# cg-tuwien/ppsurf

Hardware: AMD Instinct MI355X
Metric: occupancy query-points/sec @ res=257, 50NN (higher is better)
Workload: dtype f16x3

## Files before the change

ppsurf_amd/csrc/pps_decode.hip:

```cpp
#include <cstdlib>
#include "pps_common.h"
#include "../../include/ppsurf_amd.h"

using namespace pps;

#define NT 256
#define NW (NT / 64)
#define WG_PER_CU (512 / NT)
#ifndef PPS_PRIO
#define PPS_PRIO 1
#endif
#ifndef PPS_PRIO_PN
#define PPS_PRIO_PN 1
#endif
#define CH4 2048

template <int CHUNK_F4_NEXT, int NTH = NT, class F>
__device__ __forceinline__ void stream_step(const f32x4* __restrict__ gnext, f32x4*& cur, f32x4*& nxt, F&& compute) {
    chunk_copy_async<CHUNK_F4_NEXT / NTH, NTH>(gnext, nxt);
    compute((const f32x4*)cur);
    stream_wait();
    wg_barrier();
    f32x4* t = cur; cur = nxt; nxt = t;
}
// ... 773 lines not shown

#define PB_NBIAS (128 + 64 + 4096)
#define PB_LDS_BYTES (2 * CH4 * 16 + 4096 * 4)

__global__ __launch_bounds__(NT, 2) void pointnet_stn_fc_kernel(const float* __restrict__ gin, int64_t Q,
                                                                const float* __restrict__ wpack, const float* __restrict__ bias,
                                                                float* __restrict__ trans2, const int* __restrict__ gate) {
    if (gate_closed(gate)) return;
    float* bias_l = (float*)((f32x4*)pps_smem + 2 * CH4);
    const f32x4* bias4 = (const f32x4*)bias_l;
    const f32x4* wg = (const f32x4*)wpack;
    const int lane = lane_id(), wave = threadIdx.x >> 6, n = lane & 15, g = lane >> 4;

    lds_fill(bias_l, bias + 192, 4096);
    const f32x4* bias_g = (const f32x4*)bias;
    f32x4 *cur, *nxt;
    stream_begin<CH4>(wg, cur, nxt);

    const int ntiles = (int)((Q + NW * 16 - 1) / (NW * 16));
    int first, count, stride;
    xcd_tile_range(ntiles, first, count, stride);
    for (int it = 0; it < count; ++it) {
        const TileRow q = tile_row(first + it * stride, wave, n, Q);
        f32x4 a[16], h[8], u[4];
        {
            const f32x4* src = (const f32x4*)(gin + q.c * 256) + g;
#pragma unroll
            for (int bb = 0; bb < 16; ++bb) a[bb] = src[4 * bb];
        }
#pragma unroll
        for (int c = 0; c < 4; ++c)
            stream_step<CH4>(wg + (c + 1) * CH4, cur, nxt,
                           [&](const f32x4* w) { dense_blocks<16, 2, 1>(a, &h[2 * c], w, bias_g + 8 * c, lane); });
        stream_step<CH4>(wg + 5 * CH4, cur, nxt, [&](const f32x4* w) { dense_blocks<8, 4, 1>(h, u, w, bias_g + 32, lane); });
        f32x4* dst = (f32x4*)(trans2 + q.c * 4096) + g;
#pragma unroll 1
        for (int c = 0; c < 32; ++c) {
            f32x4 o[8];
            const f32x4* gn = (c + 1 < 32) ? wg + (6 + c) * CH4 : wg;
            stream_step<CH4>(gn, cur, nxt, [&](const f32x4* w) { dense_blocks<4, 8, 0>(u, o, w, bias4 + 32 * c, lane); });
            if (q.valid) {
#pragma unroll
                for (int j = 0; j < 8; ++j) dst[4 * (8 * c + j)] = o[j];
            }
        }
    }
}

__device__ __forceinline__ void stn_head_h(const float* __restrict__ grow, const f32x4* wg, const f32x4* after, const f32x4* __restrict__ bias_g,
                                           f32x4*& cur, f32x4*& nxt, int lane, float& amax, HiLo (&u)[2]) {
    HiLo ah[8], h[4];
    {
        f32x4 a[16];
        const f32x4* src = (const f32x4*)grow + (lane >> 4);
#pragma unroll
        for (int bb = 0; bb < 16; ++bb) a[bb] = src[4 * bb];
#pragma unroll
        for (int kb = 0; kb < 8; ++kb) ah[kb] = split_f16_r(amax, a[2 * kb], a[2 * kb + 1]);
    }
#pragma unroll
    for (int c = 0; c < 4; ++c)
        stream_step<CH4>(wg + (c + 1) * CH4, cur, nxt, [&](const f32x4* w) {
            dense_blocks_f16x3<8, 2, 1>(ah, (const half8*)w, bias_g + 8 * c, lane, [&](int, const f32x4& o0, const f32x4& o1) { h[c] = split_f16_r(amax, o0, o1); }); });
    stream_step<CH4>(after, cur, nxt, [&](const f32x4* w) {
        dense_blocks_f16x3<4, 4, 1>(h, (const half8*)w, bias_g + 32, lane, [&](int i, const f32x4& o0, const f32x4& o1) { u[i] = split_f16_r(amax, o0, o1); }); });
}

__global__ __launch_bounds__(NT, 2) void pointnet_stn_fc_h_kernel(const float* __restrict__ gin, int64_t Q, const f32x4* __restrict__ w16,
                                                                  const float* __restrict__ bias, half8* __restrict__ trans2h, int* __restrict__ range) {
    float amax = 0.f;
    float* bias_l = (float*)((f32x4*)pps_smem + 2 * CH4);
    const f32x4* bias4 = (const f32x4*)bias_l;
    const f32x4* wg = w16;
    const int lane = lane_id(), wave = threadIdx.x >> 6, n = lane & 15, g = lane >> 4;

    lds_fill(bias_l, bias + 192, 4096);
    const f32x4* bias_g = (const f32x4*)bias;
    f32x4 *cur, *nxt;
    stream_begin<CH4>(wg, cur, nxt);
    const int ntiles = (int)((Q + NW * 16 - 1) / (NW * 16));
    int first, count, stride;
    xcd_tile_range(ntiles, first, count, stride);
    for (int it = 0; it < count; ++it) {
        const TileRow q = tile_row(first + it * stride, wave, n, Q);
        HiLo u[2];
        stn_head_h(gin + q.c * 256, wg, wg + 5 * CH4, bias_g, cur, nxt, lane, amax, u);
        half8* dst = trans2h + q.c * 1024 + g;
#pragma unroll 1
        for (int c = 0; c < 32; ++c) {
            const f32x4* gn = (c + 1 < 32) ? wg + (6 + c) * CH4 : wg;
            stream_step<CH4>(gn, cur, nxt, [&](const f32x4* w) {
                dense_blocks_f16x3<2, 8, 0, false>(u, (const half8*)w, bias4 + 32 * c, lane, [&](int i, const f32x4& o0, const f32x4& o1) {
                    const int a = 2 * c + (i >> 1), kb = i & 1;
                    const HiLo v = split_f16_r(amax, o0, o1);
                    if (q.valid) {
                        half8* d = dst + (((a >> 4) * 2 + kb) * 2) * 64 + 4 * (a & 15);
                        d[0] = v.hi;
                        d[64] = v.lo;
                    }
                }); });
        }
    }
    range_commit(amax, range);
}

#define PC_W_XYZ 256
#define PC_NBIAS (576 + 256 + 4)
#define PC_WFLOATS (4096 + 8192)
#define PC_LDS_BYTES ((PC_WFLOATS + PC_W_XYZ + PC_NBIAS) * 4)

struct PhaseC {
    const f32x4 *w_c0b, *w_c2, *bias4, *u4;
    const float* xyz_l;
};
template <int NTH>
__device__ __forceinline__ PhaseC phase_c_setup(const float* __restrict__ wpack, const f32x4* __restrict__ wdense, const float* __restrict__ bias) {
    f32x4* w_l = (f32x4*)pps_smem;
    float* xyz_l = (float*)(w_l + PC_WFLOATS / 4);
    float* bias_l = xyz_l + PC_W_XYZ;
    for (int i = threadIdx.x; i < PC_WFLOATS / 4; i += NTH) w_l[i] = wdense[i];
    lds_fill(xyz_l, wpack, PC_W_XYZ);
    lds_fill(bias_l, bias, PC_NBIAS);
    const f32x4* bias4 = (const f32x4*)bias_l;
    return PhaseC{w_l, w_l + 1024, bias4, bias4 + 144, xyz_l};
}

template <bool H>
__device__ __forceinline__ void feat_rows_query(const float* __restrict__ patches, int64_t q, int P, int ntile_rows, const half8 (&th)[4][2],
                                                const half8 (&tl)[4][2], const f32x4 (&tf)[4][4], const PhaseC& pc, float s0, float& amax, int lane,
                                                float* __restrict__ xbar) {
    const int n = lane & 15, g = lane >> 4;
    const f32x4 *bias4 = pc.bias4, *u4 = pc.u4, *w_c0b = pc.w_c0b, *w_c2 = pc.w_c2;
    const float* xyz_l = pc.xyz_l;
    f32x4 acc[8];
    float mrun = -INFINITY, ssum = 0.f;
#pragma unroll
    for (int bb = 0; bb < 8; ++bb) acc[bb] = f32x4{0.f, 0.f, 0.f, 0.f};
    for (int rb = 0; rb < ntile_rows; ++rb) {
        const int rowi = rb * 16 + n;
        const bool valid = rowi < P;
        const int rowc = valid ? rowi : P - 1;
        const float coord = (g < 3) ? patches[(q * P + rowc) * 3 + g] : 0.f;
        f32x4 x0[4], y[8];
#pragma unroll
        for (int bb = 0; bb < 4; ++bb) x0[bb] = bias4[4 * bb + g];
        xyz_blocks<4>(coord, x0, xyz_l, lane);
        relu_blocks<4>(x0);
        __builtin_amdgcn_s_setprio(PPS_PRIO_PN);
        float s = 0.f;
        if (H) {
            HiLo a[2], b[2];
            a[0] = split_f16_r(amax, x0[0], x0[1]);
            a[1] = split_f16_r(amax, x0[2], x0[3]);
            dense_blocks_f16x3<2, 4, 1>(a, (const half8*)w_c0b, bias4 + 16, lane, [&](int i, const f32x4& o0, const f32x4& o1) { b[i] = split_f16_r(amax, o0, o1); });
#pragma unroll
            for (int ob = 0; ob < 4; ++ob) {
                f32x4 o = bias4[32 + 4 * ob + g], c = {0.f, 0.f, 0.f, 0.f};
#pragma unroll
                for (int kb = 0; kb < 2; ++kb) {
                    o = __builtin_amdgcn_mfma_f32_16x16x32_f16(th[ob][kb], b[kb].hi, o, 0, 0, 0);
                    c = __builtin_amdgcn_mfma_f32_16x16x32_f16(th[ob][kb], b[kb].lo, c, 0, 0, 0);
                    c = __builtin_amdgcn_mfma_f32_16x16x32_f16(tl[ob][kb], b[kb].hi, c, 0, 0, 0);
                }
                o += c;
#pragma unroll
                for (int r = 0; r < 4; ++r) x0[ob][r] = fmaxf(o[r], 0.f);
            }
            a[0] = split_f16_r(amax, x0[0], x0[1]);
            a[1] = split_f16_r(amax, x0[2], x0[3]);
            dense_blocks_f16x3<2, 8, 1>(a, (const half8*)w_c2, bias4 + 48, lane, [&](int i, const f32x4& o0, const f32x4& o1) {
                const f32x4 w0 = u4[4 * (2 * i) + g], w1 = u4[4 * (2 * i + 1) + g];
#pragma unroll
                for (int r = 0; r < 4; ++r) s += w0[r] * o0[r] + w1[r] * o1[r];
                y[2 * i] = o0;
                y[2 * i + 1] = o1;
            });
        } else {
            f32x4 x1[4];
            dense_blocks<4, 4, 1>(x0, x1, w_c0b, bias4 + 16, lane);
#pragma unroll
            for (int ob = 0; ob < 4; ++ob) {
                f32x4 o = bias4[32 + 4 * ob + g];
#pragma unroll
                for (int kb = 0; kb < 4; ++kb) {
                    o = __builtin_amdgcn_mfma_f32_16x16x4f32(tf[ob][kb].x, x1[kb].x, o, 0, 0, 0);
                    o = __builtin_amdgcn_mfma_f32_16x16x4f32(tf[ob][kb].y, x1[kb].y, o, 0, 0, 0);
                    o = __builtin_amdgcn_mfma_f32_16x16x4f32(tf[ob][kb].z, x1[kb].z, o, 0, 0, 0);
                    o = __builtin_amdgcn_mfma_f32_16x16x4f32(tf[ob][kb].w, x1[kb].w, o, 0, 0, 0);
                }
#pragma unroll
                for (int r = 0; r < 4; ++r) x0[ob][r] = fmaxf(o[r], 0.f);
            }
            dense_blocks<4, 8, 1>(x0, y, w_c2, bias4 + 48, lane);
#pragma unroll
            for (int bb = 0; bb < 8; ++bb) {
                const f32x4 w4 = u4[4 * bb + g];
#pragma unroll
                for (int r = 0; r < 4; ++r) s += w4[r] * y[bb][r];
            }
        }
        __builtin_amdgcn_s_setprio(0);
        s += shfl_xor_f32(s, 16);
        s += shfl_xor_f32(s, 32);
        s += s0;
        const float mblk = row16_max(valid ? s : -INFINITY);
        const float mnew = fmaxf(mrun, mblk);
        const float scale = __expf(mrun - mnew);
        const float en = valid ? __expf(s - mnew) : 0.f;
        mrun = mnew;
        ssum = ssum * scale + en;
#pragma unroll
        for (int bb = 0; bb < 8; ++bb)
#pragma unroll
            for (int r = 0; r < 4; ++r) acc[bb][r] = acc[bb][r] * scale + en * y[bb][r];
    }
    const float inv = 1.f / row16_sum(ssum);
    rows16_sum_transposed8(acc, lane);
    if (n < 8) ((f32x4*)(xbar + q * 128))[4 * n + g] = acc[0] * inv;
}

template <bool H>
__device__ __forceinline__ void pointnet_feat_rows_body(const float* __restrict__ patches, const float* __restrict__ trans2,
                                                        int64_t Q, int P, const float* __restrict__ wpack,
                                                        const f32x4* __restrict__ wdense, const float* __restrict__ bias,
                                                        float* __restrict__ xbar, int* __restrict__ flag) {
    if (!H && gate_closed(flag)) return;
    float amax = 0.f;
    const int lane = lane_id(), wave = threadIdx.x >> 6, n = lane & 15, g = lane >> 4;
    const PhaseC pc = phase_c_setup<PNT>(wpack, wdense, bias);
    wg_barrier();
    const float s0 = ((const float*)pc.bias4)[576 + 256];
    const int ntile_rows = (P + 15) / 16;

    const int ntiles = (int)((Q + PNW - 1) / PNW);
    int first, count, stride;
    xcd_tile_range(ntiles, first, count, stride);
    for (int it = 0; it < count; ++it) {
        const int64_t q = (int64_t)(first + it * stride) * PNW + wave;
        if (q >= Q) continue;
        half8 th[4][2], tl[4][2];
        f32x4 tf[4][4];
        if (H) {
            const half8* tq = (const half8*)trans2 + q * 1024 + 4 * n + g;
#pragma unroll
            for (int ob = 0; ob < 4; ++ob)
#pragma unroll
                for (int kb = 0; kb < 2; ++kb) { th[ob][kb] = tq[((ob * 2 + kb) * 2) * 64]; tl[ob][kb] = tq[((ob * 2 + kb) * 2 + 1) * 64]; }
        } else {
            const f32x4* tq = (const f32x4*)(trans2 + q * 4096);
#pragma unroll
            for (int ob = 0; ob < 4; ++ob)
#pragma unroll
                for (int kb = 0; kb < 4; ++kb) tf[ob][kb] = tq[(16 * ob + n) * 16 + 4 * kb + g];
        }
        feat_rows_query<H>(patches, q, P, ntile_rows, th, tl, tf, pc, s0, amax, lane, xbar);
    }
    if (H) range_commit(amax, flag);
}
template <bool H>
__global__ __launch_bounds__(PNT, 2) void pointnet_feat_rows_kernel(const float* __restrict__ patches, const float* __restrict__ trans2,
                                                                    int64_t Q, int P, const float* __restrict__ wpack,
                                                                    const f32x4* __restrict__ wdense, const float* __restrict__ bias,
                                                                    float* __restrict__ xbar, int* __restrict__ flag) {
    pointnet_feat_rows_body<H>(patches, trans2, Q, P, wpack, wdense, bias, xbar, flag);
}
template <>
PPS_PLAIN_F32
__global__ __launch_bounds__(PNT, 2) void pointnet_feat_rows_kernel<true>(const float* __restrict__ patches, const float* __restrict__ trans2,
                                                                          int64_t Q, int P, const float* __restrict__ wpack,
                                                                          const f32x4* __restrict__ wdense, const float* __restrict__ bias,
                                                                          float* __restrict__ xbar, int* __restrict__ flag) {
    pointnet_feat_rows_body<true>(patches, trans2, Q, P, wpack, wdense, bias, xbar, flag);
}

#define PH_LDS_BYTES (2 * CH4 * 16)
__global__ __launch_bounds__(NT, 2) void pointnet_stn_head_h_kernel(const float* __restrict__ gin, int64_t Q, const f32x4* __restrict__ w16,
                                                                    const float* __restrict__ bias, half8* __restrict__ uh, int* __restrict__ range) {
    float amax = 0.f;
    const f32x4* wg = w16;
    const int lane = lane_id(), wave = threadIdx.x >> 6, n = lane & 15, g = lane >> 4;
    const f32x4* bias_g = (const f32x4*)bias;
    f32x4 *cur, *nxt;
    stream_begin<CH4>(wg, cur, nxt);
    const int ntiles = (int)((Q + NW * 16 - 1) / (NW * 16));
    int first, count, stride;
    xcd_tile_range(ntiles, first, count, stride);
    for (int it = 0; it < count; ++it) {
        const TileRow q = tile_row(first + it * stride, wave, n, Q);
        HiLo u[2];
        stn_head_h(gin + q.c * 256, wg, wg, bias_g, cur, nxt, lane, amax, u);
        if (q.valid) {
            half8* dst = uh + q.c * 16 + g;
#pragma unroll
            for (int kb = 0; kb < 2; ++kb) { dst[(2 * kb) * 4] = u[kb].hi; dst[(2 * kb + 1) * 4] = u[kb].lo; }
        }
    }
    range_commit(amax, range);
}

#define PF_NT 512
#define PF_QSTRIDE 257
#define PF_BUF (8 * PF_QSTRIDE)
#define PF_LDS_BYTES (PC_LDS_BYTES + 3 * PF_BUF * 16)
PPS_PLAIN_F32
__global__ __launch_bounds__(PF_NT, 2) void pointnet_fc3_feat_rows_kernel(const float* __restrict__ patches, const half8* __restrict__ uh,
                                                                          int64_t Q, int P, const f32x4* __restrict__ wfc,
                                                                          const float* __restrict__ bias_fc, const float* __restrict__ wpack,
                                                                          const f32x4* __restrict__ wdense, const float* __restrict__ bias,
                                                                          float* __restrict__ xbar, int* __restrict__ flag) {
    float amax = 0.f;
    half8* ex = (half8*)(pps_smem + PC_LDS_BYTES);
    const int lane = lane_id(), wave = __builtin_amdgcn_readfirstlane(threadIdx.x >> 6), n = lane & 15, g = lane >> 4;
    const PhaseC pc = phase_c_setup<PF_NT>(wpack, wdense, bias);
    const float s0 = bias[576 + 256];
    const int ntile_rows = (P + 15) / 16;
    const f32x4* w3 = wfc + 5 * CH4;
    const f32x4* b3 = (const f32x4*)(bias_fc + 192);
    half8* ex_w = ex + (n < 8 ? n * PF_QSTRIDE : PF_BUF + (n - 8) * PF_QSTRIDE) + 8 * wave + g;
    const half8* ex_r = ex + wave * PF_QSTRIDE + 4 * n + g;
    const half8* ex_r2 = ex_r + PF_BUF;

    const int ntiles = (int)((Q + 15) / 16);
    int first, count, stride;
    xcd_tile_range(ntiles, first, count, stride);
    const f32x4 tf[4][4] = {};
    for (int it = 0; it < count; ++it) {
        const int64_t q0 = (int64_t)(first + it * stride) * 16;
        half8 th[4][2], tl[4][2], th2[2][2], tl2[2][2];
        {
            const int64_t qc = q0 + n < Q ? q0 + n : Q - 1;
            HiLo u[2];
#pragma unroll
            for (int kb = 0; kb < 2; ++kb) { u[kb].hi = uh[qc * 16 + (2 * kb) * 4 + g]; u[kb].lo = uh[qc * 16 + (2 * kb + 1) * 4 + g]; }
#pragma unroll
            for (int ob = 0; ob < 4; ++ob) {
                wg_barrier();
                const int c = 8 * ob + wave;
                const half8* wc = (const half8*)(w3 + c * CH4);
                asm volatile("" : "+s"(wc));
                dense_blocks_f16x3<2, 8, 0, false>(u, wc, b3 + 32 * c, lane, [&](int i, const f32x4& o0, const f32x4& o1) {
                    const HiLo v = split_f16_r(amax, o0, o1);
                    half8* d = ex_w + (n >= 8 ? (ob & 1) * PF_BUF : 0) + ((i & 1) * 2) * 64 + 4 * (i >> 1);
                    d[0] = v.hi;
                    d[64] = v.lo;
                });
                wg_barrier();
#pragma unroll
                for (int kb = 0; kb < 2; ++kb) {
                    th[ob][kb] = ex_r[(2 * kb) * 64];
                    tl[ob][kb] = ex_r[(2 * kb + 1) * 64];
                    if (ob < 2) {
                        th2[ob][kb] = ex_r2[ob * PF_BUF + (2 * kb) * 64];
                        tl2[ob][kb] = ex_r2[ob * PF_BUF + (2 * kb + 1) * 64];
                    }
                }
            }
        }
        if (q0 + wave < Q) feat_rows_query<true>(patches, q0 + wave, P, ntile_rows, th, tl, tf, pc, s0, amax, lane, xbar);
        if (q0 + wave + 8 < Q) {
#pragma unroll
            for (int kb = 0; kb < 2; ++kb) {
#pragma unroll
                for (int ob = 0; ob < 2; ++ob) {
                    th[ob][kb] = th2[ob][kb];
                    tl[ob][kb] = tl2[ob][kb];
                    th[2 + ob][kb] = ex_r2[ob * PF_BUF + (2 * kb) * 64];
                    tl[2 + ob][kb] = ex_r2[ob * PF_BUF + (2 * kb + 1) * 64];
                }
            }
            feat_rows_query<true>(patches, q0 + wave + 8, P, ntile_rows, th, tl, tf, pc, s0, amax, lane, xbar);
        }
    }
    range_commit(amax, flag);
}

#define TL_NBIAS (256 + 256 + 32)
#define TL_LDS_BYTES (2 * CH4 * 16 + TL_NBIAS * 4)

__global__ __launch_bounds__(NT, 2) void decode_tail_kernel(const float* __restrict__ pooled, const float* __restrict__ xbar, int64_t Q,
                                                            const float* __restrict__ wpack, const float* __restrict__ bias,
                                                            float* __restrict__ logits, float* __restrict__ occ, int* __restrict__ gate) {
    if (gate_closed(gate)) return;
    if (gate != nullptr && blockIdx.x == 0 && threadIdx.x == 0) atomicAdd(gate + 1, 1);
    float* bias_l = (float*)((f32x4*)pps_smem + 2 * CH4);
    const f32x4* bias4 = (const f32x4*)bias_l;
    const f32x4* wg = (const f32x4*)wpack;
    const int lane = lane_id(), wave = threadIdx.x >> 6, n = lane & 15, g = lane >> 4;

    lds_fill(bias_l, bias, TL_NBIAS);
    f32x4 *cur, *nxt;
    stream_begin<CH4>(wg, cur, nxt);

    const int ntiles = (int)((Q + NW * 16 - 1) / (NW * 16));
    int first, count, stride;
    xcd_tile_range(ntiles, first, count, stride);
    for (int it = 0; it < count; ++it) {
        const TileRow q = tile_row(first + it * stride, wave, n, Q);
        f32x4 p[16], x[8], h[16];
        {
            const f32x4* sp = (const f32x4*)(pooled + q.c * 256) + g;
            const f32x4* sx = (const f32x4*)(xbar + q.c * 128) + g;
#pragma unroll
            for (int bb = 0; bb < 16; ++bb) p[bb] = sp[4 * bb];
#pragma unroll
            for (int bb = 0; bb < 8; ++bb) x[bb] = sx[4 * bb];
        }
#pragma unroll
        for (int c = 0; c < 8; ++c)
            stream_step<CH4>(wg + (c + 1) * CH4, cur, nxt,
                           [&](const f32x4* w) { dense_blocks<16, 2, 0>(p, &h[2 * c], w, bias4 + 8 * c, lane); });
#pragma unroll
        for (int c = 0; c < 4; ++c)
            stream_step<CH4>(wg + (c + 9) * CH4, cur, nxt,
                           [&](const f32x4* w) { dense_blocks<8, 4, 1, 1>(x, &h[4 * c], w, bias4, lane); });
#pragma unroll
        for (int c = 0; c < 8; ++c)
            stream_step<CH4>(wg + (c + 13) * CH4, cur, nxt,
                           [&](const f32x4* w) { dense_blocks<16, 2, 1>(h, &p[2 * c], w, bias4 + 64 + 8 * c, lane); });
        f32x4 o[2];
        stream_step<CH4>(wg, cur, nxt, [&](const f32x4* w) { dense_blocks<16, 2, 0>(p, o, w, bias4 + 128, lane); });
        store_logits(o[0], q, g, logits, occ);
    }
}

PPS_PLAIN_F32
__global__ __launch_bounds__(NT, 2) void decode_tail_h_kernel(const float* __restrict__ pooled, const float* __restrict__ xbar, int64_t Q,
                                                              const f32x4* __restrict__ w16, const float* __restrict__ bias,
                                                              float* __restrict__ logits, float* __restrict__ occ, int* __restrict__ range) {
    float amax = 0.f;
    float* bias_l = (float*)((f32x4*)pps_smem + 2 * CH4);
    const f32x4* bias4 = (const f32x4*)bias_l;
    const f32x4* wg = w16;
    const int lane = lane_id(), wave = threadIdx.x >> 6, n = lane & 15, g = lane >> 4;

    lds_fill(bias_l, bias, TL_NBIAS);
    f32x4 *cur, *nxt;
    stream_begin<CH4>(wg, cur, nxt);

    const int ntiles = (int)((Q + NW * 16 - 1) / (NW * 16));
    int first, count, stride;
    xcd_tile_range(ntiles, first, count, stride);
    for (int it = 0; it < count; ++it) {
        const TileRow q = tile_row(first + it * stride, wave, n, Q);
        HiLo p[8], x[4];
        {
            const f32x4* sp = (const f32x4*)(pooled + q.c * 256) + g;
            const f32x4* sx = (const f32x4*)(xbar + q.c * 128) + g;
#pragma unroll
            for (int kb = 0; kb < 8; ++kb) p[kb] = split_f16_r(amax, sp[4 * (2 * kb)], sp[4 * (2 * kb + 1)]);
#pragma unroll
            for (int kb = 0; kb < 4; ++kb) x[kb] = split_f16_r(amax, sx[4 * (2 * kb)], sx[4 * (2 * kb + 1)]);
        }
        HiLo y[8];
#pragma unroll
        for (int c = 0; c < 8; ++c) {
            f32x4 h[2];
            stream_step<CH4 / 2>(wg + c * 3072 + 2048, cur, nxt, [&](const f32x4* w) {
                dense_blocks_f16x3<8, 2, 0>(p, (const half8*)w, bias4 + 8 * c, lane, [&](int, const f32x4& o0, const f32x4& o1) { h[0] = o0; h[1] = o1; }); });
            stream_step<CH4>(c + 1 < 8 ? wg + (c + 1) * 3072 : wg + 24576, cur, nxt, [&](const f32x4* w) {
                dense_blocks_f16x3<4, 2, 1, true, true>(x, (const half8*)w, bias4, lane, [&](int, const f32x4& o0, const f32x4& o1) { y[c] = split_f16_r(amax, o0, o1); }, h); });
        }
#pragma unroll
        for (int c = 0; c < 8; ++c)
            stream_step<CH4>(wg + 24576 + (c + 1) * 2048, cur, nxt, [&](const f32x4* w) {
                dense_blocks_f16x3<8, 2, 1>(y, (const half8*)w, bias4 + 64 + 8 * c, lane, [&](int, const f32x4& o0, const f32x4& o1) { p[c] = split_f16_r(amax, o0, o1); }); });
        f32x4 o[2];
        stream_step<CH4>(wg, cur, nxt, [&](const f32x4* w) {
            dense_blocks_f16x3<8, 2, 0>(p, (const half8*)w, bias4 + 128, lane, [&](int, const f32x4& o0, const f32x4& o1) { o[0] = o0; o[1] = o1; }); });
        store_logits(o[0], q, g, logits, occ);
    }
    range_commit(amax, range);
}

static int g_cu_count = 0;
static int cu_count() {
    if (g_cu_count == 0) {
        int dev = 0;
        hipDeviceProp_t prop;
        if (hipGetDevice(&dev) != hipSuccess || hipGetDeviceProperties(&prop, dev) != hipSuccess) return -1;
        g_cu_count = prop.multiProcessorCount;
    }
    return g_cu_count;
}

static int chip_wgs(int per_cu) {
    const int cus = cu_count();
    return (cus > 0 ? cus : 256) * per_cu;
}

static int grid_for(int64_t ntiles, int wgs = chip_wgs(WG_PER_CU)) {
    return (int)(ntiles < wgs ? (ntiles > 0 ? ntiles : 1) : wgs);
}

template <auto Kernel, class... Args>
static int launch(int grid, int threads, int lds, void* stream, Args... args) {
    static const bool once = lds > 0 && hipFuncSetAttribute((const void*)Kernel, hipFuncAttributeMaxDynamicSharedMemorySize, lds) == hipSuccess;
    (void)once;
    hipLaunchKernelGGL(Kernel, dim3(grid), dim3(threads), lds, (hipStream_t)stream, args...);
    return hipGetLastError() == hipSuccess ? PPS_OK : PPS_ERR_LAUNCH;
}

struct PnSplit { int64_t q_packed; int grid_packed, grid_rest, rest_mode; };
static PnSplit pn_split(int64_t q, int p) {
    const PatchPacking pk = patch_packing(p);
    PnSplit sp;
    const int wgs = chip_wgs(PN_WG_PER_CU);
    const int64_t per_round = (int64_t)wgs * PNW * pk.qg;
    sp.q_packed = pk.packed ? (q / per_round) * per_round : 0;
    if (pk.packed && getenv("PPS_PN_FORCE_PACK")) sp.q_packed = q;
    sp.grid_packed = wgs;
    sp.rest_mode = pk.packed ? 2 : 0;
    sp.grid_rest = grid_for((q - sp.q_packed + PNW - 1) / PNW, wgs);
    return sp;
}

template <bool H>
static int launch_stn_rows(const float* patches, int64_t q, int p, const float* wpack, const void* wdense, const float* bias, float* g,
                           int* flag, void* stream) {
    const PnSplit sp = pn_split(q, p);
    const char* tiles_env = getenv("PPS_STN_TILES");
    const int tmax = (tiles_env && atoi(tiles_env) == 2) ? 2 : 3;
    int rc = PPS_OK;
    if (sp.q_packed > 0)
        rc = launch<pointnet_stn_rows_kernel<H>>(sp.grid_packed, PNT, PA_LDS_BYTES, stream, patches, sp.q_packed, p, 1, tmax, wpack,
                                                 (const f32x4*)wdense, bias, g, flag);
    if (rc == PPS_OK && q > sp.q_packed)
        rc = launch<pointnet_stn_rows_kernel<H>>(sp.grid_rest, PNT, PA_LDS_BYTES, stream, patches + sp.q_packed * p * 3, q - sp.q_packed, p,
                                                 sp.rest_mode, tmax, wpack, (const f32x4*)wdense, bias, g + sp.q_packed * 256, flag);
    return rc;
}

template <bool H>
static int launch_feat_rows(const float* patches, const float* trans2, int64_t q, int p, const float* wpack, const void* wdense,
                            const float* bias, float* xbar, int* flag, void* stream) {
    return launch<pointnet_feat_rows_kernel<H>>(grid_for((q + PNW - 1) / PNW, chip_wgs(PN_WG_PER_CU)), PNT, PC_LDS_BYTES, stream, patches, trans2, q,
                                                p, wpack, (const f32x4*)wdense, bias, xbar, flag);
}

static int interp_pool_f32_impl(const float* G, const float* pts, const float* query, const int64_t* idx, int64_t q, int k,
                                const float* wpack, const float* bias, float* pooled, const int* gate, void* stream) {
    if (q < 0 || k < 1 || k > 64) return PPS_ERR_ARG;
    if (q == 0) return PPS_OK;
    if (!G || !pts || !query || !idx || !wpack || !bias || !pooled) return PPS_ERR_ARG;
    return launch<interp_pool_kernel>(grid_for((q + NW / 4 - 1) / (NW / 4)), NT, IP_LDS_BYTES, stream, G, pts, query, idx, q, k, wpack, bias, pooled,
                                      gate);
}

static int stn_fc_f32_impl(const float* g, int64_t q, const float* wpack, const float* bias, float* trans2, const int* gate, void* stream) {
    if (q < 0) return PPS_ERR_ARG;
    if (q == 0) return PPS_OK;
    if (!g || !wpack || !bias || !trans2) return PPS_ERR_ARG;
    return launch<pointnet_stn_fc_kernel>(grid_for((q + NW * 16 - 1) / (NW * 16)), NT, PB_LDS_BYTES, stream, g, q, wpack, bias, trans2, gate);
}

static int decode_tail_f32_impl(const float* pooled, const float* xbar, int64_t q, const float* wpack, const float* bias,
                                float* logits, float* occ, int* gate, void* stream) {
    if (q < 0) return PPS_ERR_ARG;
    if (q == 0) return PPS_OK;
    if (!pooled || !xbar || !wpack || !bias || !logits) return PPS_ERR_ARG;
    return launch<decode_tail_kernel>(grid_for((q + NW * 16 - 1) / (NW * 16)), NT, TL_LDS_BYTES, stream, pooled, xbar, q, wpack, bias, logits, occ,
                                      gate);
}

extern "C" {

int pps_abi_version(void) { return 2; }

int pps_device_cu_count(void) { return cu_count(); }

int pps_rows_dense256_f32(const float* in, int64_t rs, int64_t cs, int64_t m, const float* wpack, const float* bias,
                          float* out, void* stream) {
    if (m < 0) return PPS_ERR_ARG;
    if (m == 0) return PPS_OK;
    if (!in || !wpack || !bias || !out) return PPS_ERR_ARG;
    if (cs == 1 && (rs % 4) != 0) return PPS_ERR_ARG;
    return launch<rows_dense256_kernel>(grid_for((m + NW * 16 - 1) / (NW * 16)), NT, RD_LDS_BYTES, stream, in, rs, cs, m, wpack, bias, out);
}

int pps_interp_pool_f32(const float* G, const float* pts, const float* query, const int64_t* idx, int64_t q, int k,
                        const float* wpack, const float* bias, float* pooled, void* stream) {
    return interp_pool_f32_impl(G, pts, query, idx, q, k, wpack, bias, pooled, nullptr, stream);
}

int pps_interp_pool_f16x3(const float* G, const float* pts, const float* query, const int64_t* idx, int64_t q, int k,
                          const float* wxyz, const void* w16, const float* bias, float* pooled, int32_t* range_flag, void* stream) {
    if (q < 0 || k < 1 || k > 64) return PPS_ERR_ARG;
    if (q == 0) return PPS_OK;
    if (!G || !pts || !query || !idx || !wxyz || !w16 || !bias || !pooled) return PPS_ERR_ARG;
    const int grid = grid_for((q + IH_NW / 4 - 1) / (IH_NW / 4), chip_wgs(IH_WG_PER_CU));
    return launch<interp_pool_f16x3_kernel>(grid, IH_NT, IH_LDS_BYTES, stream, G, pts, query, idx, q, k, wxyz, (const f32x4*)w16, bias, pooled,
                                            (int*)range_flag);
}

int pps_interp_small_f32(const float* G, const float* pts, const float* query, const int64_t* idx, int64_t q, int k, int c,
                         const float* wpack, const float* bias, const float* wtail, int nout, float* out, void* stream) {
    if (q < 0 || k < 1 || k > 64 || (c != 32 && c != 64) || nout < 1 || nout > IS_MAX_OUT) return PPS_ERR_ARG;
    if (q == 0) return PPS_OK;
    if (!G || !pts || !query || !idx || !wpack || !bias || !wtail || !out) return PPS_ERR_ARG;
    const int grid = grid_for(q, chip_wgs(8));
    if (c == 32) return launch<interp_small_kernel<2, false>>(grid, IS_NT, 0, stream, G, pts, query, idx, q, k, wpack, nullptr, bias, wtail, nout, out, nullptr);
    return launch<interp_small_kernel<4, false>>(grid, IS_NT, 0, stream, G, pts, query, idx, q, k, wpack, nullptr, bias, wtail, nout, out, nullptr);
}

int pps_interp_small_f16x3(const float* G, const float* pts, const float* query, const int64_t* idx, int64_t q, int k, int c,
                           const float* wpack, const void* w16, const float* bias, const float* wtail, int nout, float* out, int* guard,
                           void* stream) {
    if (q < 0 || k < 1 || k > 64 || (c != 32 && c != 64) || nout < 1 || nout > IS_MAX_OUT) return PPS_ERR_ARG;
    if (q == 0) return PPS_OK;
    if (!G || !pts || !query || !idx || !wpack || !w16 || !bias || !wtail || !out || !guard) return PPS_ERR_ARG;
    const int grid = grid_for(q, chip_wgs(8));
    if (hipMemsetAsync(guard, 0, sizeof(int), (hipStream_t)stream) != hipSuccess) return PPS_ERR_LAUNCH;
    const float* wh = (const float*)w16;
    int rc;
    if (c == 32) {
        rc = launch<interp_small_kernel<2, true>>(grid, IS_NT, 0, stream, G, pts, query, idx, q, k, wpack, wh, bias, wtail, nout, out, guard);
        if (rc == PPS_OK) rc = launch<interp_small_kernel<2, false>>(grid, IS_NT, 0, stream, G, pts, query, idx, q, k, wpack, nullptr, bias, wtail, nout, out, guard);
    } else {
        rc = launch<interp_small_kernel<4, true>>(grid, IS_NT, 0, stream, G, pts, query, idx, q, k, wpack, wh, bias, wtail, nout, out, guard);
        if (rc == PPS_OK) rc = launch<interp_small_kernel<4, false>>(grid, IS_NT, 0, stream, G, pts, query, idx, q, k, wpack, nullptr, bias, wtail, nout, out, guard);
    }
    return rc;
}

int pps_pointnet_stn_rows_f32(const float* patches, int64_t q, int p, const float* wpack, const float* bias, float* g,
                              void* stream) {
    if (q < 0 || p < 1) return PPS_ERR_ARG;
    if (q == 0) return PPS_OK;
    if (!patches || !wpack || !bias || !g) return PPS_ERR_ARG;
    return launch_stn_rows<false>(patches, q, p, wpack, wpack + PA_W_XYZ, bias, g, nullptr, stream);
}

int pps_pointnet_stn_fc_f32(const float* g, int64_t q, const float* wpack, const float* bias, float* trans2, void* stream) {
    return stn_fc_f32_impl(g, q, wpack, bias, trans2, nullptr, stream);
}

int pps_pointnet_feat_rows_f32(const float* patches, const float* trans2, int64_t q, int p, const float* wpack,
                               const float* bias, float* xbar, void* stream) {
    if (q < 0 || p < 1) return PPS_ERR_ARG;
    if (q == 0) return PPS_OK;
    if (!patches || !trans2 || !wpack || !bias || !xbar) return PPS_ERR_ARG;
    return launch_feat_rows<false>(patches, trans2, q, p, wpack, wpack + PC_W_XYZ, bias, xbar, nullptr, stream);
}

int pps_pointnet_f16x3(const float* patches, int64_t q, int p, const float* const* weights ,
                       const void* const* w16, float* g, float* trans2, float* xbar, int32_t* range_flag, void* const* events, void* stream) {
    if (q < 0 || p < 1) return PPS_ERR_ARG;
    if (q == 0) return PPS_OK;
    if (!patches || !weights || !w16 || !w16[0] || !w16[1] || !w16[2] || !g || !trans2 || !xbar) return PPS_ERR_ARG;
    int* range = (int*)range_flag;
    auto mark = [&](int i) { if (events && events[i]) hipEventRecord((hipEvent_t)events[i], (hipStream_t)stream); };
    int rc = launch_stn_rows<true>(patches, q, p, weights[0], w16[0], weights[1], g, range, stream);
    mark(0);
    if (rc != PPS_OK) return rc;
    const int head_grid = grid_for((q + NW * 16 - 1) / (NW * 16));
    const char* fused_env = getenv("PPS_PN_FUSED");
    const bool fused = !(fused_env && fused_env[0] == '0' && fused_env[1] == 0);
    rc = fused ? launch<pointnet_stn_head_h_kernel>(head_grid, NT, PH_LDS_BYTES, stream, g, q, (const f32x4*)w16[1], weights[3], (half8*)trans2, range)
               : launch<pointnet_stn_fc_h_kernel>(head_grid, NT, PB_LDS_BYTES, stream, g, q, (const f32x4*)w16[1], weights[3], (half8*)trans2, range);
    mark(1);
    if (rc != PPS_OK) return rc;
    rc = fused ? launch<pointnet_fc3_feat_rows_kernel>(grid_for((q + 15) / 16, chip_wgs(1)), PF_NT, PF_LDS_BYTES, stream, patches, (const half8*)trans2,
                                                       q, p, (const f32x4*)w16[1], weights[3], weights[4], (const f32x4*)w16[2], weights[5], xbar, range)
               : launch_feat_rows<true>(patches, trans2, q, p, weights[4], w16[2], weights[5], xbar, range, stream);
    mark(2);
    return rc;
}

int pps_decode_tail_f32(const float* pooled, const float* xbar, int64_t q, const float* wpack, const float* bias,
                        float* logits, float* occ, void* stream) {
    return decode_tail_f32_impl(pooled, xbar, q, wpack, bias, logits, occ, nullptr, stream);
}

int pps_decode_tail_f16x3(const float* pooled, const float* xbar, int64_t q, const void* w16, const float* bias, float* logits, float* occ,
                          int32_t* range_flag, void* stream) {
// ... 78 lines not shown
```

Baseline: 13.49 million.

## Software-pipeline fc3 weight loads through a register ring in fused feat-rows kernel

Replaces the dense_blocks_f16x3 call in the fc3 stage with a hand-unrolled 32-step MFMA loop. Weight and bias fragments are prefetched PF_DEPTH steps ahead into a register ring, and the first steps for the next tile are issued before the loop back-edge. The aim is to hide global weight-load latency behind the MFMA work and the feat_rows phase. In exchange it raises register pressure (ring of half8 fragments plus biases) under launch_bounds(512,2), and it reissues the weights from global memory on every tile.

```diff
diff --git a/ppsurf_amd/csrc/pps_decode.hip b/ppsurf_amd/csrc/pps_decode.hip
--- a/ppsurf_amd/csrc/pps_decode.hip
+++ b/ppsurf_amd/csrc/pps_decode.hip
@@ -1099,6 +1099,45 @@
 #define PF_QSTRIDE 257
 #define PF_BUF (8 * PF_QSTRIDE)
 #define PF_LDS_BYTES (PC_LDS_BYTES + 3 * PF_BUF * 16)
+#ifndef PF_DEPTH
+#define PF_DEPTH 2
+#endif
+#define PF_STEPS 32
+#define PF_RING (2 * PF_DEPTH + 1)
+#define PF_PIN_VMEM 0
+struct Fc3Step { half8 h0, l0, h1, l1; };
+template <class T>
+__device__ __forceinline__ const __attribute__((address_space(1))) T* opaque_global(const T* p) {
+    asm volatile("" : "+s"(p));
+    return (const __attribute__((address_space(1))) T*)p;
+}
+__device__ __forceinline__ void fc3_request(int s, const half8* __restrict__ w3, const f32x4* __restrict__ b3, int wave, int lane, Fc3Step& f,
+                                            f32x4 (&b)[2]) {
+    s &= PF_STEPS - 1;
+    const int p = (s >> 1) & 3, kb = s & 1;
+    int c = 8 * (s >> 3) + wave;
+    asm volatile("" : "+s"(c));
+    if (kb == 0) {
+        const auto* bc = opaque_global(b3 + 32 * c + 8 * p) + ((unsigned)lane >> 4);
+        b[0] = bc[0];
+        b[1] = bc[4];
+    }
+    const auto* w = opaque_global(w3 + c * CH4 + p * 512 + kb * 128) + (unsigned)lane;
+    f.h0 = w[0];
+    f.l0 = w[64];
+    f.h1 = w[256];
+    f.l1 = w[320];
+}
+
+__device__ __forceinline__ void fc3_request_u(int tile, const half8* __restrict__ uh, int64_t Q, int lane, HiLo (&u)[2]) {
+    const int64_t qn = (int64_t)tile * 16 + (lane & 15), qc = qn < Q ? qn : Q - 1;
+    const half8* pu = uh + qc * 16 + (lane >> 4);
+    asm volatile("" : "+v"(pu));
+    const auto* src = (const __attribute__((address_space(1))) half8*)pu;
+#pragma unroll
+    for (int kb = 0; kb < 2; ++kb) { u[kb].hi = src[(2 * kb) * 4]; u[kb].lo = src[(2 * kb + 1) * 4]; }
+}
+
 PPS_PLAIN_F32
 __global__ __launch_bounds__(PF_NT, 2) void pointnet_fc3_feat_rows_kernel(const float* __restrict__ patches, const half8* __restrict__ uh,
                                                                           int64_t Q, int P, const f32x4* __restrict__ wfc,
@@ -1111,7 +1150,7 @@
     const PhaseC pc = phase_c_setup<PF_NT>(wpack, wdense, bias);
     const float s0 = bias[576 + 256];
     const int ntile_rows = (P + 15) / 16;
-    const f32x4* w3 = wfc + 5 * CH4;
+    const half8* w3 = (const half8*)(wfc + 5 * CH4);
     const f32x4* b3 = (const f32x4*)(bias_fc + 192);
     half8* ex_w = ex + (n < 8 ? n * PF_QSTRIDE : PF_BUF + (n - 8) * PF_QSTRIDE) + 8 * wave + g;
     const half8* ex_r = ex + wave * PF_QSTRIDE + 4 * n + g;
@@ -1121,34 +1160,53 @@
     int first, count, stride;
     xcd_tile_range(ntiles, first, count, stride);
     const f32x4 tf[4][4] = {};
+    Fc3Step fr[PF_RING];
+    f32x4 fb[PF_DEPTH + 1][2];
+#pragma unroll
+    for (int s = 0; s < 2 * PF_DEPTH; ++s) fc3_request(s, w3, b3, wave, lane, fr[s % PF_RING], fb[(s >> 1) % (PF_DEPTH + 1)]);
     for (int it = 0; it < count; ++it) {
         const int64_t q0 = (int64_t)(first + it * stride) * 16;
         half8 th[4][2], tl[4][2], th2[2][2], tl2[2][2];
         {
-            const int64_t qc = q0 + n < Q ? q0 + n : Q - 1;
             HiLo u[2];
-#pragma unroll
-            for (int kb = 0; kb < 2; ++kb) { u[kb].hi = uh[qc * 16 + (2 * kb) * 4 + g]; u[kb].lo = uh[qc * 16 + (2 * kb + 1) * 4 + g]; }
-#pragma unroll
-            for (int ob = 0; ob < 4; ++ob) {
-                wg_barrier();
-                const int c = 8 * ob + wave;
-                const half8* wc = (const half8*)(w3 + c * CH4);
-                asm volatile("" : "+s"(wc));
-                dense_blocks_f16x3<2, 8, 0, false>(u, wc, b3 + 32 * c, lane, [&](int i, const f32x4& o0, const f32x4& o1) {
-                    const HiLo v = split_f16_r(amax, o0, o1);
+            fc3_request_u(first + it * stride, uh, Q, lane, u);
+            f32x4 m0, m1, c0, c1;
+#pragma unroll
+            for (int s = 0; s < PF_STEPS; ++s) {
+                const int ob = s >> 3, i = (s >> 1) & 3, kb = s & 1;
+                if ((s & 7) == 0) wg_barrier();
+                if (s + 2 * PF_DEPTH < PF_STEPS)
+                    fc3_request(s + 2 * PF_DEPTH, w3, b3, wave, lane, fr[(s + 2 * PF_DEPTH) % PF_RING], fb[((s >> 1) + PF_DEPTH) % (PF_DEPTH + 1)]);
+                __builtin_amdgcn_sched_barrier(PF_PIN_VMEM);
+                const Fc3Step& a = fr[s % PF_RING];
+                if (kb == 0) {
+                    m0 = fb[(s >> 1) % (PF_DEPTH + 1)][0];
+                    m1 = fb[(s >> 1) % (PF_DEPTH + 1)][1];
+                    c0 = f32x4{0.f, 0.f, 0.f, 0.f};
+                    c1 = c0;
+                }
+                m0 = __builtin_amdgcn_mfma_f32_16x16x32_f16(a.h0, u[kb].hi, m0, 0, 0, 0);
+                m1 = __builtin_amdgcn_mfma_f32_16x16x32_f16(a.h1, u[kb].hi, m1, 0, 0, 0);
+                c0 = __builtin_amdgcn_mfma_f32_16x16x32_f16(a.h0, u[kb].lo, c0, 0, 0, 0);
+                c1 = __builtin_amdgcn_mfma_f32_16x16x32_f16(a.h1, u[kb].lo, c1, 0, 0, 0);
+                c0 = __builtin_amdgcn_mfma_f32_16x16x32_f16(a.l0, u[kb].hi, c0, 0, 0, 0);
+                c1 = __builtin_amdgcn_mfma_f32_16x16x32_f16(a.l1, u[kb].hi, c1, 0, 0, 0);
+                if (kb == 1) {
+                    const HiLo v = split_f16_r(amax, m0 + c0, m1 + c1);
                     half8* d = ex_w + (n >= 8 ? (ob & 1) * PF_BUF : 0) + ((i & 1) * 2) * 64 + 4 * (i >> 1);
                     d[0] = v.hi;
                     d[64] = v.lo;
-                });
-                wg_barrier();
-#pragma unroll
-                for (int kb = 0; kb < 2; ++kb) {
-                    th[ob][kb] = ex_r[(2 * kb) * 64];
-                    tl[ob][kb] = ex_r[(2 * kb + 1) * 64];
-                    if (ob < 2) {
-                        th2[ob][kb] = ex_r2[ob * PF_BUF + (2 * kb) * 64];
-                        tl2[ob][kb] = ex_r2[ob * PF_BUF + (2 * kb + 1) * 64];
+                }
+                if ((s & 7) == 7) {
+                    wg_barrier();
+#pragma unroll
+                    for (int k = 0; k < 2; ++k) {
+                        th[ob][k] = ex_r[(2 * k) * 64];
+                        tl[ob][k] = ex_r[(2 * k + 1) * 64];
+                        if (ob < 2) {
+                            th2[ob][k] = ex_r2[ob * PF_BUF + (2 * k) * 64];
+                            tl2[ob][k] = ex_r2[ob * PF_BUF + (2 * k + 1) * 64];
+                        }
                     }
                 }
             }
@@ -1167,6 +1225,8 @@
             }
             feat_rows_query<true>(patches, q0 + wave + 8, P, ntile_rows, th, tl, tf, pc, s0, amax, lane, xbar);
         }
+#pragma unroll
+        for (int s = 0; s < 2 * PF_DEPTH; ++s) fc3_request(PF_STEPS + s, w3, b3, wave, lane, fr[s % PF_RING], fb[(s >> 1) % (PF_DEPTH + 1)]);
     }
     range_commit(amax, flag);
 }
```

Measured after the change: 13.56 million, median of 6. Within noise of the previous version (+0.5%).
